# eudald-seeslab/mmsbm

Hardware: NVIDIA B200
Metric: rating-updates/sec (higher is better)
Workload: dtype f64

## Files before the change

mmsbm_b200/csrc/em_step.cu:

```cuda
#include <stdlib.h>

#include "common.cuh"
#include "em_internal.cuh"
#include "segment_pass.cuh"

namespace mmsbm {

constexpr int kPrThreads = 128;
constexpr int kPrBatch = 16;
constexpr int kGemmThreads = 256;
constexpr int kGemmBK = 32;
constexpr int kGemmTR = 4;

__global__ void __launch_bounds__(128) segment_fixup_kernel(const SegArgs A) {
  const int run = blockIdx.y, RNB = A.R * A.NBp;
  const int n_long = __ldg(A.sched + 2);
  const int32_t* long_seg = A.sched + 4 + 3 * A.pmax;
  const int32_t* long_slot0 = long_seg + A.lmax;
  for (int li = blockIdx.x; li < n_long; li += gridDim.x) {
    const int sg = __ldg(long_seg + li), s0 = __ldg(long_slot0 + li), s1 = __ldg(long_slot0 + li + 1);
    MMSBM_DEV_CHECK(sg >= 0 && sg < A.nseg && s0 >= 0 && s0 < s1 && s1 <= A.smax);
    const double* src = A.partial + ((size_t)run * A.smax + s0) * RNB;
    double* dst = A.wg + ((size_t)run * A.nseg + sg) * RNB;
    for (int o = threadIdx.x; o < RNB; o += blockDim.x) {
      double acc = 0.0;
      for (int k = 0; k < s1 - s0; ++k) acc += src[(size_t)k * RNB + o];
      dst[o] = acc;
    }
  }
}

__global__ void interleave_runs_kernel(const double* __restrict__ src, double* __restrict__ dst, int n_src,
                                       int n_dst, int row0, int ld, int group0, int groups, int gs) {
  const int c4 = ld >> 2;
  const size_t total = (size_t)groups * n_src * gs * c4;
  const size_t t = (size_t)blockIdx.x * blockDim.x + threadIdx.x;
  if (t >= total) return;
  const int c = (int)(t % c4);
  const int j = (int)((t / c4) % gs);
  const size_t rest = t / c4 / gs;
  const int id = (int)(rest % n_src);
  const size_t p = group0 + rest / n_src;
  const double4_t v = ldg256(src + (((size_t)(gs * p + j) * n_src + id) * ld + 4 * c));
  stg256(dst + (((p * n_dst + row0 + id) * gs + j) * ld + 4 * c), v);
}

__global__ void prep_p_kernel(const double* pr, int K, int L, int R, int ldk, int ldl, double* pw_u,
                              double* pn_u, double* pw_i, double* pn_i) {
  const int run = blockIdx.y;
  const int total = ldk * ldl * R;
  const int t = blockIdx.x * blockDim.x + threadIdx.x;
  if (t >= total) return;
  const int r = t % R, kl = t / R, lp = kl % ldl, kp = kl / ldl;
  double v = 0.0;
  if (kp < K && lp < L) v = __ldg(pr + (((size_t)run * K + kp) * L + lp) * R + r);
  const size_t base = (size_t)run * total;
  const int rnb_u = R * ldl, rnb_i = R * ldk;
  pw_u[base + (size_t)kp * rnb_u + r * ldl + lp] = v;
  pn_u[base + (size_t)(r * ldl + lp) * ldk + kp] = v;
  pw_i[base + (size_t)lp * rnb_i + r * ldk + kp] = v;
  pn_i[base + (size_t)(r * ldk + kp) * ldl + lp] = v;
}

struct GemmArgs {
  const double* A;
  const double* B;
  double* C;
  const double* own;
  const int32_t* deg;
  int M, N, Kd, lda, rg, normalize;
  int b_resident;
  int bk;
};

template <bool EPI>
__global__ void __launch_bounds__(kGemmThreads) small_gemm_kernel(const GemmArgs g) {
  constexpr int TR = kGemmTR;
  extern __shared__ __align__(32) unsigned char smem_raw[];
  const int BM = TR * g.rg, AS = g.bk + 2;
  double* Bs = reinterpret_cast<double*>(smem_raw);
  double* As = Bs + (size_t)(g.b_resident ? g.Kd : g.bk) * g.N;
  const int run = blockIdx.y;
  const int ncg = g.N >> 2, half = g.N >> 1;
  const int rgid = threadIdx.x / ncg, cg = threadIdx.x - rgid * ncg;
  const bool active = rgid < g.rg;
  const double* A = g.A + (size_t)run * g.M * g.lda;
  const double2* B2 = reinterpret_cast<const double2*>(g.B + (size_t)run * g.Kd * g.N);
  double2* Bs2 = reinterpret_cast<double2*>(Bs);
  if (g.b_resident)
    for (int t = threadIdx.x; t < (g.Kd * g.N) >> 1; t += kGemmThreads) Bs2[t] = __ldg(B2 + t);
  const int n_tiles = (g.M + BM - 1) / BM;
  for (int tile = blockIdx.x; tile < n_tiles; tile += gridDim.x) {
    const int row0 = tile * BM;
    double acc[TR][4];
#pragma unroll
    for (int i = 0; i < TR; ++i)
#pragma unroll
      for (int j = 0; j < 4; ++j) acc[i][j] = 0.0;

    for (int k0 = 0; k0 < g.Kd; k0 += g.bk) {
      const int bk = min(g.bk, g.Kd - k0);
      const int bk2 = bk >> 1;
      __syncthreads();
      for (int t = threadIdx.x; t < BM * bk2; t += kGemmThreads) {
        const int m = t / bk2, p2 = t - m * bk2;
        double2 v = make_double2(0.0, 0.0);
        if (row0 + m < g.M) v = __ldg(reinterpret_cast<const double2*>(A + (size_t)(row0 + m) * g.lda + k0) + p2);
        *reinterpret_cast<double2*>(As + m * AS + 2 * p2) = v;
      }
      if (!g.b_resident)
        for (int t = threadIdx.x; t < (bk * g.N) >> 1; t += kGemmThreads)
          Bs2[t] = __ldg(B2 + (((size_t)k0 * g.N) >> 1) + t);
      __syncthreads();
      if (active) {
        const double* ap = As + (size_t)(TR * rgid) * AS;
        const double* bp = Bs + (size_t)(g.b_resident ? k0 : 0) * g.N + 2 * cg;
        for (int kk = 0; kk < bk; kk += 2) {
          const double2 b00 = *reinterpret_cast<const double2*>(bp + (size_t)kk * g.N);
          const double2 b01 = *reinterpret_cast<const double2*>(bp + (size_t)kk * g.N + half);
          const double2 b10 = *reinterpret_cast<const double2*>(bp + (size_t)(kk + 1) * g.N);
          const double2 b11 = *reinterpret_cast<const double2*>(bp + (size_t)(kk + 1) * g.N + half);
#pragma unroll
          for (int i = 0; i < TR; ++i) {
            const double2 a = *reinterpret_cast<const double2*>(ap + i * AS + kk);
            acc[i][0] = fma(a.x, b00.x, acc[i][0]); acc[i][1] = fma(a.x, b00.y, acc[i][1]);
            acc[i][2] = fma(a.x, b01.x, acc[i][2]); acc[i][3] = fma(a.x, b01.y, acc[i][3]);
            acc[i][0] = fma(a.y, b10.x, acc[i][0]); acc[i][1] = fma(a.y, b10.y, acc[i][1]);
            acc[i][2] = fma(a.y, b11.x, acc[i][2]); acc[i][3] = fma(a.y, b11.y, acc[i][3]);
          }
        }
      }
    }
    if (active) {
#pragma unroll
      for (int i = 0; i < TR; ++i) {
        const int m = row0 + TR * rgid + i;
        if (m >= g.M) continue;
        const size_t off = ((size_t)run * g.M + m) * g.N + 2 * cg;
        double2 v0 = make_double2(acc[i][0], acc[i][1]), v1 = make_double2(acc[i][2], acc[i][3]);
        if (EPI) {
          const double2 o0 = __ldg(reinterpret_cast<const double2*>(g.own + off));
          const double2 o1 = __ldg(reinterpret_cast<const double2*>(g.own + off + half));
          v0.x *= o0.x; v0.y *= o0.y; v1.x *= o1.x; v1.y *= o1.y;
          if (g.normalize) {
            const double d = (double)max(__ldg(g.deg + m), 1);
            v0.x = v0.x / d; v0.y = v0.y / d; v1.x = v1.x / d; v1.y = v1.y / d;
          }
        }
        *reinterpret_cast<double2*>(g.C + off) = v0;
        *reinterpret_cast<double2*>(g.C + off + half) = v1;
      }
    }
  }
}

constexpr int kRowThreads = 256;

template <int LD, int ROWS>
__global__ void __launch_bounds__(kRowThreads) row_w_kernel(const double* __restrict__ own,
                                                            const double* __restrict__ pw,
                                                            double* __restrict__ W, int M, int RNB) {
  extern __shared__ __align__(32) unsigned char smem_raw[];
  double* Ps = reinterpret_cast<double*>(smem_raw);
  const int run = blockIdx.y;
  {
    const double2* src = reinterpret_cast<const double2*>(pw + (size_t)run * LD * RNB);
    double2* dst = reinterpret_cast<double2*>(Ps);
    for (int t = threadIdx.x; t < (LD * RNB) >> 1; t += kRowThreads) dst[t] = __ldg(src + t);
  }
  __syncthreads();
  const double* own_run = own + (size_t)run * M * LD;
  double* w_run = W + (size_t)run * M * RNB;
  for (int m0 = blockIdx.x * (kRowThreads * ROWS) + threadIdx.x; m0 < M; m0 += gridDim.x * (kRowThreads * ROWS)) {
    double o[ROWS][LD];
    int mr[ROWS];
#pragma unroll
    for (int j = 0; j < ROWS; ++j) {
      mr[j] = m0 + j * kRowThreads;
      const int mc = mr[j] < M ? mr[j] : m0;
#pragma unroll
      for (int c = 0; c < LD / 4; ++c) {
        const double4_t v = ldg256(own_run + (size_t)mc * LD + 4 * c);
        o[j][4 * c] = v.x; o[j][4 * c + 1] = v.y; o[j][4 * c + 2] = v.z; o[j][4 * c + 3] = v.w;
      }
    }
    for (int ob = 0; ob < RNB; ob += 4) {
      double4_t acc[ROWS];
#pragma unroll
      for (int j = 0; j < ROWS; ++j) acc[j] = double4_t{0.0, 0.0, 0.0, 0.0};
#pragma unroll
      for (int a = 0; a < LD; ++a) {
        const double4_t p = lds32(Ps + a * RNB + ob);
#pragma unroll
        for (int j = 0; j < ROWS; ++j) {
          acc[j].x = fma(o[j][a], p.x, acc[j].x); acc[j].y = fma(o[j][a], p.y, acc[j].y);
          acc[j].z = fma(o[j][a], p.z, acc[j].z); acc[j].w = fma(o[j][a], p.w, acc[j].w);
        }
      }
#pragma unroll
      for (int j = 0; j < ROWS; ++j)
        if (mr[j] < M) stg256(w_run + (size_t)mr[j] * RNB + ob, acc[j]);
    }
  }
}

template <int LD, int ROWS, int PF>
__global__ void __launch_bounds__(kRowThreads) row_n_kernel(const double* __restrict__ G,
                                                            const double* __restrict__ pn,
                                                            const double* __restrict__ own,
                                                            const int32_t* __restrict__ deg,
                                                            double* __restrict__ out, int M, int RNB,
                                                            int normalize, const RowPublish pub) {
  extern __shared__ __align__(32) unsigned char smem_raw[];
  double* Ps = reinterpret_cast<double*>(smem_raw);
  const int run = blockIdx.y;
  double* pdst = nullptr;
  int pgs = 1, pj = 0;
  size_t pgrp = 0;
#pragma unroll
  for (int t = 0; t < 3; ++t) {
    if (pub.dst[t] != nullptr && run >= pub.gs[t] * pub.group0[t] && run < pub.gs[t] * (pub.group0[t] + pub.groups[t])) {
      pdst = pub.dst[t]; pgs = pub.gs[t]; pgrp = (size_t)(run / pub.gs[t]); pj = run % pub.gs[t];
    }
  }
  {
    const double2* src = reinterpret_cast<const double2*>(pn + (size_t)run * LD * RNB);
    double2* dst = reinterpret_cast<double2*>(Ps);
    for (int t = threadIdx.x; t < (LD * RNB) >> 1; t += kRowThreads) dst[t] = __ldg(src + t);
  }
  __syncthreads();
  const double* g_run = G + (size_t)run * M * RNB;
  const double* own_run = own + (size_t)run * M * LD;
  double* out_run = out + (size_t)run * M * LD;
  for (int m0 = blockIdx.x * (kRowThreads * ROWS) + threadIdx.x; m0 < M; m0 += gridDim.x * (kRowThreads * ROWS)) {
    double acc[ROWS][LD];
    int mr[ROWS];
    const double* grow[ROWS];
#pragma unroll
    for (int j = 0; j < ROWS; ++j) {
      mr[j] = m0 + j * kRowThreads;
      grow[j] = g_run + (size_t)(mr[j] < M ? mr[j] : m0) * RNB;
#pragma unroll
      for (int a = 0; a < LD; ++a) acc[j][a] = 0.0;
    }
    for (int ob0 = 0; ob0 < RNB; ob0 += 4 * PF) {
      double4_t gq[ROWS][PF];
#pragma unroll
      for (int j = 0; j < ROWS; ++j)
#pragma unroll
        for (int p = 0; p < PF; ++p) gq[j][p] = ldg256(grow[j] + ob0 + 4 * p);
#pragma unroll
      for (int p = 0; p < PF; ++p) {
        const int ob = ob0 + 4 * p;
        double gv[ROWS][4];
#pragma unroll
        for (int j = 0; j < ROWS; ++j) {
          gv[j][0] = gq[j][p].x; gv[j][1] = gq[j][p].y; gv[j][2] = gq[j][p].z; gv[j][3] = gq[j][p].w;
        }
#pragma unroll
        for (int i = 0; i < 4; ++i) {
#pragma unroll
          for (int c = 0; c < LD / 4; ++c) {
            const double4_t pv = lds32(Ps + (ob + i) * LD + 4 * c);
#pragma unroll
            for (int j = 0; j < ROWS; ++j) {
              acc[j][4 * c] = fma(gv[j][i], pv.x, acc[j][4 * c]);         acc[j][4 * c + 1] = fma(gv[j][i], pv.y, acc[j][4 * c + 1]);
              acc[j][4 * c + 2] = fma(gv[j][i], pv.z, acc[j][4 * c + 2]); acc[j][4 * c + 3] = fma(gv[j][i], pv.w, acc[j][4 * c + 3]);
            }
          }
        }
      }
    }
#pragma unroll
    for (int j = 0; j < ROWS; ++j) {
      if (mr[j] >= M) continue;
      double d = 1.0;
      if (normalize) d = (double)max(__ldg(deg + mr[j]), 1);
#pragma unroll
      for (int c = 0; c < LD / 4; ++c) {
        const double4_t ov = ldg256(own_run + (size_t)mr[j] * LD + 4 * c);
        double4_t v{acc[j][4 * c] * ov.x, acc[j][4 * c + 1] * ov.y, acc[j][4 * c + 2] * ov.z, acc[j][4 * c + 3] * ov.w};
        if (normalize) { v.x = v.x / d; v.y = v.y / d; v.z = v.z / d; v.w = v.w / d; }
        stg256(out_run + (size_t)mr[j] * LD + 4 * c, v);
        if (pdst) stg256(pdst + (((pgrp * pub.n_all + pub.row0 + mr[j]) * pgs + pj) * LD + 4 * c), v);
      }
    }
  }
}

struct PrArgs {
  const double* own;
  const double* g;
  double* partial;
  int nseg, NA, lda, RNB;
};

__global__ void __launch_bounds__(kPrThreads) pr_accumulate_kernel(const PrArgs A) {
  extern __shared__ __align__(32) unsigned char smem_raw[];
  double* own_s = reinterpret_cast<double*>(smem_raw);
  double* g_s = own_s + kPrBatch * A.lda;
  const int run = blockIdx.y, slab = blockIdx.x;
  const int per = (A.nseg + kPrSlabs - 1) / kPrSlabs;
  const int s0 = slab * per, s1 = min(s0 + per, A.nseg);
  const int nout = A.NA * A.RNB;
  const int ta = A.lda >> 2, tb = A.RNB >> 2, n_tiles = ta * tb;
  const double* own_run = A.own + (size_t)run * A.nseg * A.lda;
  const double* g_run = A.g + (size_t)run * A.nseg * A.RNB;
  double* dst = A.partial + ((size_t)run * kPrSlabs + slab) * nout;

  for (int tile0 = 0; tile0 < n_tiles; tile0 += kPrThreads) {
    const int tile = tile0 + threadIdx.x;
    const bool on = tile < n_tiles;
    const int a0 = on ? 4 * (tile / tb) : 0, b0 = on ? 4 * (tile % tb) : 0;
    double acc[4][4];
#pragma unroll
    for (int i = 0; i < 4; ++i)
#pragma unroll
      for (int k = 0; k < 4; ++k) acc[i][k] = 0.0;
    for (int c0 = s0; c0 < s1; c0 += kPrBatch) {
      const int nb = min(kPrBatch, s1 - c0);
      __syncthreads();
      {
        const double2* src = reinterpret_cast<const double2*>(own_run + (size_t)c0 * A.lda);
        double2* d2 = reinterpret_cast<double2*>(own_s);
        for (int t = threadIdx.x; t < (nb * A.lda) >> 1; t += kPrThreads) d2[t] = __ldg(src + t);
        src = reinterpret_cast<const double2*>(g_run + (size_t)c0 * A.RNB);
        d2 = reinterpret_cast<double2*>(g_s);
        for (int t = threadIdx.x; t < (nb * A.RNB) >> 1; t += kPrThreads) d2[t] = __ldg(src + t);
      }
      __syncthreads();
      if (on) {
        for (int sg = 0; sg < nb; ++sg) {
          const double4_t o = lds32(own_s + sg * A.lda + a0);
          const double4_t g = lds32(g_s + sg * A.RNB + b0);
          const double ov[4] = {o.x, o.y, o.z, o.w};
#pragma unroll
          for (int i = 0; i < 4; ++i) {
            acc[i][0] = fma(ov[i], g.x, acc[i][0]); acc[i][1] = fma(ov[i], g.y, acc[i][1]);
            acc[i][2] = fma(ov[i], g.z, acc[i][2]); acc[i][3] = fma(ov[i], g.w, acc[i][3]);
          }
        }
      }
    }
    if (on) {
#pragma unroll
      for (int i = 0; i < 4; ++i)
        if (a0 + i < A.NA)
          stg256(dst + (size_t)(a0 + i) * A.RNB + b0, double4_t{acc[i][0], acc[i][1], acc[i][2], acc[i][3]});
    }
  }
}

struct PrFinArgs {
  const double* partial;
  const double* pr;
  double* pr_out;
  int K, L, R, NA, NBp, transposed, normalize;
};

constexpr int kFinWarps = 8;
__global__ void __launch_bounds__(kFinWarps * 32) pr_finalize_kernel(const PrFinArgs A) {
  extern __shared__ __align__(16) unsigned char smem_raw[];
  const int run = blockIdx.y, a = blockIdx.x;
  const int RNB = A.R * A.NBp, nout = A.NA * RNB;
  double* part_s = reinterpret_cast<double*>(smem_raw);
  double* tot_s = part_s + kFinWarps * RNB;
  const int lane = threadIdx.x & 31, warp = threadIdx.x >> 5;
  const double* part = A.partial + (size_t)run * kPrSlabs * nout + (size_t)a * RNB;
  constexpr int per = kPrSlabs / kFinWarps;
  for (int o = lane; o < RNB; o += 32) {
    double acc = 0.0;
#pragma unroll 4
    for (int s = warp * per; s < (warp + 1) * per; ++s) acc += part[(size_t)s * nout + o];
    part_s[warp * RNB + o] = acc;
  }
  __syncthreads();
  for (int o = threadIdx.x; o < RNB; o += blockDim.x) {
    double acc = 0.0;
    for (int w = 0; w < kFinWarps; ++w) acc += part_s[w * RNB + o];
    tot_s[o] = acc;
  }
  __syncthreads();
  const int NB = A.transposed ? A.K : A.L;
  for (int b = threadIdx.x; b < NB; b += blockDim.x) {
    const int k = A.transposed ? b : a, l = A.transposed ? a : b;
    const size_t kl = (size_t)k * A.L + l;
    const double* prs = A.pr + ((size_t)run * A.K * A.L + kl) * A.R;
    double* dst = A.pr_out + ((size_t)run * A.K * A.L + kl) * A.R;
    double tot = 0.0;
    for (int r = 0; r < A.R; ++r) {
      const double v = tot_s[r * A.NBp + b] * prs[r];
      dst[r] = v;
      tot += v;
    }
    if (A.normalize) {
      const double d = (tot == 0.0) ? 1.0 : tot;
      for (int r = 0; r < A.R; ++r) dst[r] = dst[r] / d;
    }
  }
}

__global__ void finalize_eta_kernel(double* eta, const int32_t* deg, int n_items, int ldl, int L,
                                    size_t total) {
  size_t t = (size_t)blockIdx.x * blockDim.x + threadIdx.x;
  if (t >= total) return;
  int col = (int)(t % ldl);
  size_t row = t / ldl;
  int item = (int)(row % n_items);
  if (col < L) eta[t] = eta[t] / (double)max(__ldg(deg + item), 1);
}

__global__ void finalize_pr_kernel(double* pr, int KL_total, int R) {
  int t = blockIdx.x * blockDim.x + threadIdx.x;
  if (t >= KL_total) return;
  double* row = pr + (size_t)t * R;
  double tot = 0.0;
  for (int r = 0; r < R; ++r) tot += row[r];
  const double d = (tot == 0.0) ? 1.0 : tot;
  for (int r = 0; r < R; ++r) row[r] = row[r] / d;
}

struct PassShape { int G, CH, UN, MINB; };

int env_int(const char* name, int dflt) {
  const char* v = getenv(name);
  return (v && *v) ? atoi(v) : dflt;
}

int sm_count() {
  static int cached[64] = {0};
  int dev = 0;
  if (cudaGetDevice(&dev) != cudaSuccess || dev < 0 || dev >= 64) return 148;
  if (cached[dev] == 0) {
    int n = 0;
    if (cudaDeviceGetAttribute(&n, cudaDevAttrMultiProcessorCount, dev) != cudaSuccess || n <= 0) n = 148;
    cached[dev] = n;
  }
// ... 29 lines not shown
static bool pairs_enabled(int NBp, int R, int n_runs) {
  return n_runs >= 2 && NBp <= 32 && seg_smem_bytes(R, NBp, 2) <= kMaxSmemBytes && env_int("MMSBM_PAIR", 1) != 0;
}

static int g_reserved_ctas = 0;
void set_reserved_ctas(int n) { g_reserved_ctas = n > 0 ? n : 0; }

static unsigned grid_x_for(const SegArgs& a, int ctas_per_sm) {
  if (!a.counters) return (unsigned)((a.pmax + a.segs_per_cta - 1) / a.segs_per_cta);
  int64_t resident = (int64_t)sm_count() * ctas_per_sm - g_reserved_ctas;
  if (resident < 1) resident = 1;
  const int64_t want = (a.pmax + kWarps - 1) / kWarps;
  return (unsigned)(want < resident ? want : resident);
}

static bool hexa_enabled(int NBp, int R, int n_runs) {
  return n_runs >= 6 && NBp == 20 && seg_smem_bytes(R, NBp, 6) <= kMaxSmemBytes && env_int("MMSBM_HEXA", 1) != 0;
}

RunPlan plan_runs(int NBp, int R, int n_runs, bool hexa_table) {
  RunPlan p{0, 0, 0, 0};
  if (hexa_table && hexa_enabled(NBp, R, n_runs)) p.hexas = n_runs / 6;
  p.single_from = 6 * p.hexas;
  if (pairs_enabled(NBp, R, n_runs - p.single_from)) {
    p.pairs = (n_runs - p.single_from) / 2;
    p.pair_group0 = p.single_from / 2;
    p.single_from += 2 * p.pairs;
  }
  return p;
}

static int launch_segment_pass_impl(SegArgs a, const double* nbr_pairs, const double* nbr_hexa,
                                    int64_t n_ratings, int n_runs, cudaStream_t st) {
  const double avg_degree = (double)n_ratings / (double)a.nseg;
  PassShape sh = choose_shape(a.NBp, avg_degree);
  const int un_e = env_int("MMSBM_UN", 0), occ_e = env_int("MMSBM_OCC", 0);
  const RunPlan plan = plan_runs(a.NBp, a.R, n_runs, nbr_hexa != nullptr);
  const int single_from = plan.single_from;
  if (plan.hexas > 0) {
    const int hexas = plan.hexas;
    SegArgs p = a;
    p.nbr = nbr_hexa;
    p.run_base = 0;
    p.grp_base = 0;
    p.segs_per_cta = segs_per_cta_for(a.pmax, n_ratings, hexas);
    const unsigned gx = grid_x_for(p, occ_e > 0 ? occ_e : 3);
    if (p.counters) a.counters += hexas;
    const size_t smem = seg_smem_bytes(a.R, a.NBp, 6);
    int rc = MMSBM_ERANGE;
    if (un_e > 0 || occ_e > 0)
      rc = launch_segment_pass_hexa(p, sh.G, un_e > 0 ? un_e : 3, occ_e > 0 ? occ_e : 3, dim3(gx, hexas), smem, st);
    if (rc == MMSBM_ERANGE) rc = launch_segment_pass_hexa(p, sh.G, 3, 3, dim3(gx, hexas), smem, st);
    if (rc) {
      if (rc == MMSBM_ERANGE) set_error("no six-run segment-pass variant for G=%d", sh.G);
      return rc;
    }
    if (single_from == n_runs && plan.pairs == 0) return 0;
  }
  if (plan.pairs > 0) {
    MMSBM_REQUIRE(nbr_pairs, MMSBM_EINVAL, "segment pass: the table of run pairs is missing");
    const int pairs = plan.pairs;
    SegArgs p = a;
    p.nbr = nbr_pairs;
    p.run_base = 6 * plan.hexas;
    p.grp_base = plan.pair_group0;
    p.counters = a.counters;
    p.segs_per_cta = segs_per_cta_for(a.pmax, n_ratings, pairs);
    const unsigned gx = grid_x_for(p, occ_e > 0 ? occ_e : 3);
    if (p.counters) a.counters += pairs;
    const size_t smem = seg_smem_bytes(a.R, a.NBp, 2);
    int UN = (sh.G == 1) ? 2 : 3, MINB = 3;
    int rc = MMSBM_ERANGE;
    if (un_e > 0 || occ_e > 0)
      rc = launch_segment_pass_pair(p, sh.G, un_e > 0 ? un_e : UN, occ_e > 0 ? occ_e : MINB, dim3(gx, pairs), smem, st);
    if (rc == MMSBM_ERANGE) rc = launch_segment_pass_pair(p, sh.G, UN, MINB, dim3(gx, pairs), smem, st);
    if (rc == MMSBM_ERANGE && sh.G == 1) rc = launch_segment_pass_pair(p, sh.G, 2, 3, dim3(gx, pairs), smem, st);
    if (rc) {
      if (rc == MMSBM_ERANGE) set_error("no paired segment-pass variant for G=%d", sh.G);
      return rc;
    }
  }
  if (single_from == n_runs) return 0;
  a.run_base = single_from;
  a.segs_per_cta = segs_per_cta_for(a.pmax, n_ratings, n_runs - single_from);
  const unsigned gx = grid_x_for(a, occ_e > 0 ? occ_e : sh.MINB);
  const dim3 grid(gx, n_runs - single_from);
  const size_t smem = seg_smem_bytes(a.R, a.NBp, 1);
  MMSBM_REQUIRE(smem <= kMaxSmemBytes, MMSBM_ERANGE,
                "segment pass needs %zu bytes of shared memory (R=%d, row stride %d)", smem, a.R, a.NBp);
  auto go = [&](const PassShape& p) {
    switch (p.CH) {
      case 1: return launch_segment_pass_ch1(a, p.G, p.UN, p.MINB, grid, smem, st);
      case 2: return launch_segment_pass_ch2(a, p.G, p.UN, p.MINB, grid, smem, st);
      case 4: return launch_segment_pass_ch4(a, p.G, p.UN, p.MINB, grid, smem, st);
      default: return launch_segment_pass_ch8(a, p.G, p.UN, p.MINB, grid, smem, st);
    }
  };
  if (un_e > 0 || occ_e > 0) {
    PassShape alt = sh;
    if (un_e > 0) alt.UN = un_e;
    if (occ_e > 0) alt.MINB = occ_e;
    const int rc = go(alt);
    if (rc != MMSBM_ERANGE) return rc;
  }
  const int rc = go(sh);
  if (rc == MMSBM_ERANGE) set_error("no segment-pass variant for G=%d CH=%d UN=%d", sh.G, sh.CH, sh.UN);
  return rc;
}

int launch_segment_pass_and_fixup(SegArgs a, const double* nbr_pairs, const double* nbr_hexa,
                                  int64_t n_ratings, int n_runs, cudaStream_t st, bool no_long_segments) {
  int rc = launch_segment_pass_impl(a, nbr_pairs, nbr_hexa, n_ratings, n_runs, st);
  if (rc) return rc;
  if (no_long_segments) return 0;
  const int64_t fix_ctas = 4 * sm_count();
  const unsigned gx = (unsigned)(a.lmax < fix_ctas ? a.lmax : fix_ctas);
  segment_fixup_kernel<<<dim3(gx, n_runs), 128, 0, st>>>(a);
  MMSBM_LAUNCH_CHECK("segment_fixup_kernel");
  return 0;
}

template <bool EPI>
static int launch_gemm(GemmArgs g, int n_runs, cudaStream_t st) {
  const int ncg = g.N / 4;
  MMSBM_REQUIRE(g.N % 4 == 0 && g.Kd % 4 == 0 && ncg >= 1 && ncg <= kGemmThreads, MMSBM_ERANGE,
                "small gemm: N=%d Kd=%d not supported (N <= 1024, multiples of 4)", g.N, g.Kd);
  int rg = kGemmThreads / ncg;
  if (rg > 32) rg = 32;
  g.rg = rg;
  const int BM = kGemmTR * rg;
  g.bk = kGemmBK;
  size_t smem = ((size_t)g.Kd * g.N + (size_t)BM * (g.bk + 2)) * 8;
  g.b_resident = smem <= 200 * 1024;
  if (!g.b_resident) {
    auto slab_bytes = [&](int bk) { return ((size_t)bk * g.N + (size_t)BM * (bk + 2)) * 8; };
    while (g.bk > 4 && slab_bytes(g.bk) > kMaxSmemBytes) g.bk -= 4;
    smem = slab_bytes(g.bk);
  }
  MMSBM_REQUIRE(smem <= kMaxSmemBytes, MMSBM_ERANGE,
                "small gemm needs %zu bytes of shared memory (K*L*R too large)", smem);
  auto kern = small_gemm_kernel<EPI>;
  MMSBM_CUDA(cudaFuncSetAttribute(kern, cudaFuncAttributeMaxDynamicSharedMemorySize, (int)smem));
  const int n_tiles = (g.M + BM - 1) / BM;
  int per_run = (sm_count() * 3 + n_runs - 1) / n_runs;
  if (per_run > n_tiles) per_run = n_tiles;
  if (per_run < 1) per_run = 1;
  kern<<<dim3(per_run, n_runs), kGemmThreads, smem, st>>>(g);
  MMSBM_LAUNCH_CHECK("small_gemm_kernel");
  return 0;
}

int launch_w(const double* own, const double* pw, double* W, int M, int LD, int RNB, int n_runs,
             cudaStream_t st) {
  const size_t smem = (size_t)LD * RNB * 8;
  const int rows_env = env_int("MMSBM_ROWS", 2);
#define MMSBM_ROW_W(LDv)                                                                        \
  if (LD == LDv && smem <= 200 * 1024) {                                                        \
    constexpr int kRows = (LDv <= 24) ? 2 : 1;             \
    const bool two = kRows == 2 && rows_env == 2;                                               \
    auto kern = two ? row_w_kernel<LDv, kRows> : row_w_kernel<LDv, 1>;                          \
    const int per = kRowThreads * (two ? 2 : 1);                                                \
    const int gx = min((M + per - 1) / per, sm_count() * 2);                                           \
    MMSBM_CUDA(cudaFuncSetAttribute(kern, cudaFuncAttributeMaxDynamicSharedMemorySize, (int)smem)); \
    kern<<<dim3(gx, n_runs), kRowThreads, smem, st>>>(own, pw, W, M, RNB);                      \
    MMSBM_LAUNCH_CHECK("row_w_kernel");                                                         \
    return 0;                                                                                   \
  }
  MMSBM_ROW_W(4) MMSBM_ROW_W(8) MMSBM_ROW_W(12) MMSBM_ROW_W(16) MMSBM_ROW_W(20) MMSBM_ROW_W(24)
  MMSBM_ROW_W(28) MMSBM_ROW_W(32)
#undef MMSBM_ROW_W
  GemmArgs g{own, pw, W, nullptr, nullptr, M, RNB, LD, LD, 0, 0, 0, kGemmBK};
  return launch_gemm<false>(g, n_runs, st);
}

int launch_n(const double* G, const double* pn, const double* own, const int32_t* deg, double* out,
             int M, int LD, int RNB, int normalize, int n_runs, cudaStream_t st, const RowPublish* publish) {
  const size_t smem = (size_t)LD * RNB * 8;
  RowPublish pub{};
  if (publish) pub = *publish;
  const int rows_env = env_int("MMSBM_ROWS_N", 1);
  int pf = env_int("MMSBM_ROWN_PF", 5);
  if (pf != 1 && pf != 2 && pf != 5) pf = 1;
  if ((RNB / 4) % pf != 0) pf = ((RNB / 4) % 2 == 0 && pf != 1) ? 2 : 1;
#define MMSBM_ROW_N_GO(kern, two)                                                               \
  {                                                                                             \
    const int per = kRowThreads * ((two) ? 2 : 1);                                              \
    const int gx = min((M + per - 1) / per, sm_count() * 2);                                    \
    MMSBM_CUDA(cudaFuncSetAttribute(kern, cudaFuncAttributeMaxDynamicSharedMemorySize, (int)smem)); \
    kern<<<dim3(gx, n_runs), kRowThreads, smem, st>>>(G, pn, own, deg, out, M, RNB, normalize, pub); \
    MMSBM_LAUNCH_CHECK("row_n_kernel");                                                         \
    return 0;                                                                                   \
  }
#define MMSBM_ROW_N(LDv)                                                                        \
  if (LD == LDv && smem <= 200 * 1024) {                                                        \
    constexpr int kRows = (LDv <= 24) ? 2 : 1;         \
    const bool two = kRows == 2 && rows_env == 2;                                               \
    if (two) MMSBM_ROW_N_GO((row_n_kernel<LDv, kRows, 1>), true)                                \
    if (pf == 5) MMSBM_ROW_N_GO((row_n_kernel<LDv, 1, 5>), false)                               \
    if (pf == 2) MMSBM_ROW_N_GO((row_n_kernel<LDv, 1, 2>), false)                               \
    MMSBM_ROW_N_GO((row_n_kernel<LDv, 1, 1>), false)                                            \
  }
  MMSBM_ROW_N(4) MMSBM_ROW_N(8) MMSBM_ROW_N(12) MMSBM_ROW_N(16) MMSBM_ROW_N(20) MMSBM_ROW_N(24)
  MMSBM_ROW_N(28) MMSBM_ROW_N(32)
#undef MMSBM_ROW_N_GO
#undef MMSBM_ROW_N
  GemmArgs g{G, pn, out, own, deg, M, LD, RNB, RNB, 0, normalize, 0, kGemmBK};
  int rc = launch_gemm<true>(g, n_runs, st);
  if (rc || !publish) return rc;
  for (int t = 0; t < 3; ++t)
    if (pub.dst[t] && (rc = launch_interleave(out, pub.dst[t], M, pub.n_all, pub.row0, LD, pub.group0[t],
                                              pub.groups[t], pub.gs[t], st)))
      return rc;
  return 0;
}

int launch_prep_p(const double* pr, int K, int L, int R, int ldk, int ldl, int n_runs, double* pw_u,
                  double* pn_u, double* pw_i, double* pn_i, cudaStream_t st) {
  const int total = ldk * ldl * R;
  prep_p_kernel<<<dim3((total + 255) / 256, n_runs), 256, 0, st>>>(pr, K, L, R, ldk, ldl, pw_u, pn_u, pw_i, pn_i);
  MMSBM_LAUNCH_CHECK("prep_p_kernel");
  return 0;
}

int launch_interleave(const double* src, double* dst, int n_src, int n_dst, int row0, int ld, int group0,
                      int groups, int gs, cudaStream_t st) {
  const size_t tot = (size_t)groups * n_src * gs * (ld / 4);
  if (tot == 0) return 0;
  interleave_runs_kernel<<<(unsigned)((tot + 255) / 256), 256, 0, st>>>(src, dst, n_src, n_dst, row0, ld,
                                                                        group0, groups, gs);
  MMSBM_LAUNCH_CHECK("interleave_runs_kernel");
  return 0;
}

int launch_pr(const double* own, const double* g, double* partial, const double* pr, double* pr_out,
              int nseg, int NA, int lda, int NBp, int K, int L, int R, int n_runs, bool transposed,
              bool normalize, cudaStream_t st) {
  PrArgs pa{};
  pa.own = own; pa.g = g; pa.partial = partial;
  pa.nseg = nseg; pa.NA = NA; pa.lda = lda; pa.RNB = R * NBp;
  const size_t smem = (size_t)kPrBatch * (pa.lda + pa.RNB) * 8;
  MMSBM_CUDA(cudaFuncSetAttribute(pr_accumulate_kernel, cudaFuncAttributeMaxDynamicSharedMemorySize,
                                  (int)smem));
  pr_accumulate_kernel<<<dim3(kPrSlabs, n_runs), kPrThreads, smem, st>>>(pa);
  MMSBM_LAUNCH_CHECK("pr_accumulate_kernel");
  PrFinArgs fa{};
  fa.partial = partial; fa.pr = pr; fa.pr_out = pr_out;
  fa.K = K; fa.L = L; fa.R = R; fa.NA = NA; fa.NBp = NBp;
  fa.transposed = transposed ? 1 : 0;
  fa.normalize = normalize ? 1 : 0;
  const size_t fin_smem = (size_t)(kFinWarps + 1) * R * NBp * 8;
  MMSBM_CUDA(cudaFuncSetAttribute(pr_finalize_kernel, cudaFuncAttributeMaxDynamicSharedMemorySize, (int)fin_smem));
  pr_finalize_kernel<<<dim3(NA, n_runs), kFinWarps * 32, fin_smem, st>>>(fa);
  MMSBM_LAUNCH_CHECK("pr_finalize_kernel");
  return 0;
}

int launch_finalize_pr(double* pr, int kl_total, int R, cudaStream_t st) {
  finalize_pr_kernel<<<(kl_total + 127) / 128, 128, 0, st>>>(pr, kl_total, R);
  MMSBM_LAUNCH_CHECK("finalize_pr_kernel");
  return 0;
}

struct EmDims {
  int U, I, R, K, L, S, ldk, ldl, rnb_u, rnb_i;
  bool emit_items;
  int nseg_e, NA_e, NBp_e;
  size_t p_elems, wg_u_elems, wg_i_elems, partial_elems, slots_u_elems, slots_i_elems;
  size_t th2_elems, et2_elems;
  size_t et6_elems;
  size_t ctr_elems;
  int64_t lmax, smax, pmax_u, pmax_i;
};

static EmDims em_dims(int64_t N, int U, int I, int R, int K, int L, int S) {
  EmDims d;
  d.U = U; d.I = I; d.R = R; d.K = K; d.L = L; d.S = S;
  d.ldk = row_stride(K); d.ldl = row_stride(L);
  d.rnb_u = R * d.ldl; d.rnb_i = R * d.ldk;
  d.emit_items = (I <= U);
  d.nseg_e = d.emit_items ? I : U;
  d.NA_e = d.emit_items ? L : K;
  d.NBp_e = d.emit_items ? d.ldk : d.ldl;
  d.p_elems = (size_t)S * d.ldk * d.ldl * R;
  d.wg_u_elems = (size_t)S * U * d.rnb_u;
  d.wg_i_elems = (size_t)S * I * d.rnb_i;
  d.partial_elems = (size_t)S * kPrSlabs * d.NA_e * R * d.NBp_e;
  d.lmax = N / MMSBM_PIECE_LEN + 1;
  d.smax = 2 * (N / MMSBM_PIECE_LEN) + 1;
  d.pmax_u = (int64_t)U + N / MMSBM_PIECE_LEN + 1;
  d.pmax_i = (int64_t)I + N / MMSBM_PIECE_LEN + 1;
  d.slots_u_elems = (size_t)S * d.smax * d.rnb_u;
  d.slots_i_elems = (size_t)S * d.smax * d.rnb_i;
  d.th2_elems = (size_t)(S / 2) * 2 * U * d.ldk;
  d.et2_elems = (size_t)(S / 2) * 2 * I * d.ldl;
  d.et6_elems = (size_t)(S / 6) * 6 * I * d.ldl;
  d.ctr_elems = 2 * ((size_t)S + 8);
  return d;
}

static size_t em_main_bytes(const EmDims& d) {
  return 4 * align_up(d.p_elems * 8) + align_up(d.wg_u_elems * 8) + align_up(d.wg_i_elems * 8) +
         align_up(d.partial_elems * 8) + align_up(d.slots_u_elems * 8) + align_up(d.slots_i_elems * 8) +
         align_up(d.th2_elems * 8) + align_up(d.et2_elems * 8) + align_up(d.et6_elems * 8) + align_up(d.ctr_elems * 4) + 256;
}

}

using namespace mmsbm;

extern "C" int mmsbm_em_workspace_bytes(int64_t N, int32_t U, int32_t I, int32_t R, int32_t K,
                                        int32_t L, int32_t S, size_t* bytes) {
  MMSBM_REQUIRE(bytes && N >= 0 && U > 0 && I > 0 && R > 0 && K > 0 && L > 0 && S > 0, MMSBM_EINVAL,
                "mmsbm_em_workspace_bytes: bad argument");
  EmDims d = em_dims(N, U, I, R, K, L, S);
  *bytes = em_main_bytes(d);
  if (em_small_applicable(N, R, K, L, S)) *bytes += align_up(em_small_partial_elems(R, K) * 8);
  return 0;
}

struct Overlap {
  bool no_long_u = false, no_long_i = false;
  cudaStream_t side = nullptr;
  cudaEvent_t e[6] = {nullptr, nullptr, nullptr, nullptr, nullptr, nullptr};
  bool two_branch = false;
};

static int em_step_impl(const int32_t* useg, const int32_t* uadj, const int32_t* udeg,
                        const int32_t* iseg, const int32_t* iadj, const int32_t* ideg,
                        const int32_t* usched, const int32_t* isched, int64_t N, int32_t U, int32_t I, int32_t R, int32_t K, int32_t L,
                        int32_t S, const double* theta, const double* eta, const double* pr,
                        double* theta_out, double* eta_out, double* pr_out, int32_t flags,
                        void* ws, size_t ws_bytes, void* stream, cudaEvent_t* ev,
                        const Overlap* ov = nullptr) {
  MMSBM_REQUIRE(useg && uadj && udeg && iseg && iadj && ideg && usched && isched && theta && eta && pr &&
                    theta_out && eta_out && pr_out && ws, MMSBM_EINVAL, "mmsbm_em_step: null pointer");
  MMSBM_REQUIRE(N >= 0 && U > 0 && I > 0 && R > 0 && K > 0 && L > 0 && S > 0, MMSBM_EINVAL,
                "mmsbm_em_step: bad size");
  MMSBM_REQUIRE(K <= 256 && L <= 256 && R <= 31, MMSBM_ERANGE,
                "mmsbm_em_step: K, L <= 256 and R <= 31 supported (K=%d L=%d R=%d)", K, L, R);
  cudaStream_t st = static_cast<cudaStream_t>(stream);
  EmDims d = em_dims(N, U, I, R, K, L, S);
  const RunPlan plan_u = plan_runs(d.ldl, R, S, true), plan_i = plan_runs(d.ldk, R, S, false);
  Arena arena(ws, ws_bytes);
  double* pw_u = arena.take<double>(d.p_elems);
  double* pn_u = arena.take<double>(d.p_elems);
  double* pw_i = arena.take<double>(d.p_elems);
  double* pn_i = arena.take<double>(d.p_elems);
  double* wg_u = arena.take<double>(d.wg_u_elems);
  double* wg_i = arena.take<double>(d.wg_i_elems);
  double* partial = arena.take<double>(d.partial_elems);
  double* slots_u = arena.take<double>(d.slots_u_elems);
  double* slots_i = arena.take<double>(d.slots_i_elems);
  double* th2 = arena.take<double>(d.th2_elems);
  double* et2 = arena.take<double>(d.et2_elems);
  double* et6 = arena.take<double>(d.et6_elems);
  int32_t* counters = arena.take<int32_t>(d.ctr_elems);
  MMSBM_REQUIRE(pw_u && pn_u && pw_i && pn_i && wg_u && wg_i && partial && slots_u && slots_i && th2 && et2 && et6 && counters,
// ... 231 lines not shown
```

Before: 26.45 billion.

## Use FP64 DMMA tensor cores in row_w and row_n kernels

Rewrites the per-row small-GEMM kernels (own×Pw and G×Pn) to issue m8n8k4 FP64 mma.sync instead of scalar DFMA loops. The P matrices are restaged in shared memory in fragment order, and each warp processes 8-row tiles. row_n also software-prefetches the next 16-wide K chunk of G. It adds a DMMA vs DFMA microbenchmark and drops the env-selected ROWS/prefetch variants. In exchange the global accesses become narrower and strided per lane, and the shared-memory footprint grows with padding.

Measured after the change: 27.08 billion, median of 6. 2.4% higher.

```diff
diff --git a/mmsbm_b200/csrc/em_step.cu b/mmsbm_b200/csrc/em_step.cu
--- a/mmsbm_b200/csrc/em_step.cu
+++ b/mmsbm_b200/csrc/em_step.cu
@@ -154,66 +154,80 @@
   }
 }
 
+__device__ __forceinline__ void dmma(double2& d, double a, double b) {
+  asm("mma.sync.aligned.m8n8k4.row.col.f64.f64.f64.f64 {%0,%1}, {%2}, {%3}, {%0,%1};"
+      : "+d"(d.x), "+d"(d.y) : "d"(a), "d"(b));
+}
+
 constexpr int kRowThreads = 256;
-
-template <int LD, int ROWS>
+constexpr int kRowWarps = kRowThreads / 32;
+constexpr int kRowTilesW = 4;
+constexpr int kRowTilesN = 2;
+
+static size_t row_w_smem(int LD, int RNB) { return (size_t)LD * ((RNB + 7) & ~7) * 8; }
+static size_t row_n_smem(int LD, int RNB) { return (size_t)((RNB + 15) & ~15) * ((LD + 7) & ~7) * 8; }
+
+template <int LD, int TW>
 __global__ void __launch_bounds__(kRowThreads) row_w_kernel(const double* __restrict__ own,
                                                             const double* __restrict__ pw,
                                                             double* __restrict__ W, int M, int RNB) {
+  constexpr int KS = LD / 4;
   extern __shared__ __align__(32) unsigned char smem_raw[];
-  double* Ps = reinterpret_cast<double*>(smem_raw);
-  const int run = blockIdx.y;
+  double* Bs = reinterpret_cast<double*>(smem_raw);
+  const int run = blockIdx.y, lane = threadIdx.x & 31, warp = threadIdx.x >> 5;
+  const int qr = lane >> 2, qc = lane & 3;
+  const int NT = (RNB + 7) >> 3;
   {
-    const double2* src = reinterpret_cast<const double2*>(pw + (size_t)run * LD * RNB);
-    double2* dst = reinterpret_cast<double2*>(Ps);
-    for (int t = threadIdx.x; t < (LD * RNB) >> 1; t += kRowThreads) dst[t] = __ldg(src + t);
+    const double* src = pw + (size_t)run * LD * RNB;
+    for (int t = threadIdx.x; t < KS * NT * 32; t += kRowThreads) {
+      const int l = t & 31, f = t >> 5, nt = f % NT, s = f / NT, o = 8 * nt + (l >> 2);
+      Bs[t] = o < RNB ? __ldg(src + (size_t)(4 * s + (l & 3)) * RNB + o) : 0.0;
+    }
   }
   __syncthreads();
   const double* own_run = own + (size_t)run * M * LD;
   double* w_run = W + (size_t)run * M * RNB;
-  for (int m0 = blockIdx.x * (kRowThreads * ROWS) + threadIdx.x; m0 < M; m0 += gridDim.x * (kRowThreads * ROWS)) {
-    double o[ROWS][LD];
-    int mr[ROWS];
-#pragma unroll
-    for (int j = 0; j < ROWS; ++j) {
-      mr[j] = m0 + j * kRowThreads;
-      const int mc = mr[j] < M ? mr[j] : m0;
-#pragma unroll
-      for (int c = 0; c < LD / 4; ++c) {
-        const double4_t v = ldg256(own_run + (size_t)mc * LD + 4 * c);
-        o[j][4 * c] = v.x; o[j][4 * c + 1] = v.y; o[j][4 * c + 2] = v.z; o[j][4 * c + 3] = v.w;
+  for (int m0 = (blockIdx.x * kRowWarps + warp) * 8 * TW; m0 < M; m0 += gridDim.x * kRowWarps * 8 * TW) {
+    double a[TW][KS];
+#pragma unroll
+    for (int t = 0; t < TW; ++t) {
+      const int m = m0 + 8 * t + qr;
+#pragma unroll
+      for (int s = 0; s < KS; ++s) a[t][s] = m < M ? __ldg(own_run + (size_t)m * LD + 4 * s + qc) : 0.0;
+    }
+    for (int nt = 0; nt < NT; ++nt) {
+      double2 acc[TW];
+#pragma unroll
+      for (int t = 0; t < TW; ++t) acc[t] = make_double2(0.0, 0.0);
+#pragma unroll
+      for (int s = 0; s < KS; ++s) {
+        const double b = Bs[(s * NT + nt) * 32 + lane];
+#pragma unroll
+        for (int t = 0; t < TW; ++t) dmma(acc[t], a[t][s], b);
       }
-    }
-    for (int ob = 0; ob < RNB; ob += 4) {
-      double4_t acc[ROWS];
-#pragma unroll
-      for (int j = 0; j < ROWS; ++j) acc[j] = double4_t{0.0, 0.0, 0.0, 0.0};
-#pragma unroll
-      for (int a = 0; a < LD; ++a) {
-        const double4_t p = lds32(Ps + a * RNB + ob);
-#pragma unroll
-        for (int j = 0; j < ROWS; ++j) {
-          acc[j].x = fma(o[j][a], p.x, acc[j].x); acc[j].y = fma(o[j][a], p.y, acc[j].y);
-          acc[j].z = fma(o[j][a], p.z, acc[j].z); acc[j].w = fma(o[j][a], p.w, acc[j].w);
-        }
+      const int o = 8 * nt + 2 * qc;
+#pragma unroll
+      for (int t = 0; t < TW; ++t) {
+        const int m = m0 + 8 * t + qr;
+        if (m < M && o < RNB) *reinterpret_cast<double2*>(w_run + (size_t)m * RNB + o) = acc[t];
       }
-#pragma unroll
-      for (int j = 0; j < ROWS; ++j)
-        if (mr[j] < M) stg256(w_run + (size_t)mr[j] * RNB + ob, acc[j]);
-    }
-  }
-}
-
-template <int LD, int ROWS, int PF>
+    }
+  }
+}
+
+template <int LD, int TN>
 __global__ void __launch_bounds__(kRowThreads) row_n_kernel(const double* __restrict__ G,
                                                             const double* __restrict__ pn,
                                                             const double* __restrict__ own,
                                                             const int32_t* __restrict__ deg,
                                                             double* __restrict__ out, int M, int RNB,
                                                             int normalize, const RowPublish pub) {
+  constexpr int NT = (LD + 7) / 8;
   extern __shared__ __align__(32) unsigned char smem_raw[];
-  double* Ps = reinterpret_cast<double*>(smem_raw);
-  const int run = blockIdx.y;
+  double* Bs = reinterpret_cast<double*>(smem_raw);
+  const int run = blockIdx.y, lane = threadIdx.x & 31, warp = threadIdx.x >> 5;
+  const int qr = lane >> 2, qc = lane & 3;
+  const int KC = (RNB + 15) >> 4;
   double* pdst = nullptr;
   int pgs = 1, pj = 0;
   size_t pgrp = 0;
@@ -224,65 +238,73 @@
     }
   }
   {
-    const double2* src = reinterpret_cast<const double2*>(pn + (size_t)run * LD * RNB);
-    double2* dst = reinterpret_cast<double2*>(Ps);
-    for (int t = threadIdx.x; t < (LD * RNB) >> 1; t += kRowThreads) dst[t] = __ldg(src + t);
+    const double* src = pn + (size_t)run * LD * RNB;
+    for (int t = threadIdx.x; t < KC * 4 * NT * 32; t += kRowThreads) {
+      const int l = t & 31, f = t >> 5, nt = f % NT, cj = f / NT;
+      const int k = 16 * (cj >> 2) + 4 * (l & 3) + (cj & 3), n = 8 * nt + (l >> 2);
+      Bs[t] = (k < RNB && n < LD) ? __ldg(src + (size_t)k * LD + n) : 0.0;
+    }
   }
   __syncthreads();
   const double* g_run = G + (size_t)run * M * RNB;
   const double* own_run = own + (size_t)run * M * LD;
   double* out_run = out + (size_t)run * M * LD;
-  for (int m0 = blockIdx.x * (kRowThreads * ROWS) + threadIdx.x; m0 < M; m0 += gridDim.x * (kRowThreads * ROWS)) {
-    double acc[ROWS][LD];
-    int mr[ROWS];
-    const double* grow[ROWS];
-#pragma unroll
-    for (int j = 0; j < ROWS; ++j) {
-      mr[j] = m0 + j * kRowThreads;
-      grow[j] = g_run + (size_t)(mr[j] < M ? mr[j] : m0) * RNB;
-#pragma unroll
-      for (int a = 0; a < LD; ++a) acc[j][a] = 0.0;
-    }
-    for (int ob0 = 0; ob0 < RNB; ob0 += 4 * PF) {
-      double4_t gq[ROWS][PF];
-#pragma unroll
-      for (int j = 0; j < ROWS; ++j)
-#pragma unroll
-        for (int p = 0; p < PF; ++p) gq[j][p] = ldg256(grow[j] + ob0 + 4 * p);
-#pragma unroll
-      for (int p = 0; p < PF; ++p) {
-        const int ob = ob0 + 4 * p;
-        double gv[ROWS][4];
-#pragma unroll
-        for (int j = 0; j < ROWS; ++j) {
-          gv[j][0] = gq[j][p].x; gv[j][1] = gq[j][p].y; gv[j][2] = gq[j][p].z; gv[j][3] = gq[j][p].w;
-        }
-#pragma unroll
-        for (int i = 0; i < 4; ++i) {
-#pragma unroll
-          for (int c = 0; c < LD / 4; ++c) {
-            const double4_t pv = lds32(Ps + (ob + i) * LD + 4 * c);
-#pragma unroll
-            for (int j = 0; j < ROWS; ++j) {
-              acc[j][4 * c] = fma(gv[j][i], pv.x, acc[j][4 * c]);         acc[j][4 * c + 1] = fma(gv[j][i], pv.y, acc[j][4 * c + 1]);
-              acc[j][4 * c + 2] = fma(gv[j][i], pv.z, acc[j][4 * c + 2]); acc[j][4 * c + 3] = fma(gv[j][i], pv.w, acc[j][4 * c + 3]);
-            }
+  const double4_t zero{0.0, 0.0, 0.0, 0.0};
+  for (int m0 = (blockIdx.x * kRowWarps + warp) * 8 * TN; m0 < M; m0 += gridDim.x * kRowWarps * 8 * TN) {
+    const double* grow[TN];
+    bool live[TN];
+    double2 acc[TN][NT];
+#pragma unroll
+    for (int t = 0; t < TN; ++t) {
+      const int m = m0 + 8 * t + qr;
+      live[t] = m < M;
+      grow[t] = g_run + (size_t)(live[t] ? m : 0) * RNB + 4 * qc;
+#pragma unroll
+      for (int nt = 0; nt < NT; ++nt) acc[t][nt] = make_double2(0.0, 0.0);
+    }
+    double4_t x[TN], y[TN];
+#pragma unroll
+    for (int t = 0; t < TN; ++t) {
+      x[t] = (live[t] && 4 * qc < RNB) ? ldg256(grow[t]) : zero;
+      y[t] = zero;
+    }
+    for (int c = 0; c < KC; ++c) {
+      if (c + 1 < KC) {
+        const bool in = 16 * (c + 1) + 4 * qc < RNB;
+#pragma unroll
+        for (int t = 0; t < TN; ++t) y[t] = (live[t] && in) ? ldg256(grow[t] + 16 * (c + 1)) : zero;
+      }
+      const double* bc = Bs + (size_t)c * 4 * NT * 32 + lane;
+#pragma unroll
+      for (int j = 0; j < 4; ++j) {
+#pragma unroll
+        for (int nt = 0; nt < NT; ++nt) {
+          const double b = bc[(j * NT + nt) * 32];
+#pragma unroll
+          for (int t = 0; t < TN; ++t) {
+            const double a = j == 0 ? x[t].x : j == 1 ? x[t].y : j == 2 ? x[t].z : x[t].w;
+            dmma(acc[t][nt], a, b);
           }
         }
       }
-    }
-#pragma unroll
-    for (int j = 0; j < ROWS; ++j) {
-      if (mr[j] >= M) continue;
+#pragma unroll
+      for (int t = 0; t < TN; ++t) x[t] = y[t];
+    }
+#pragma unroll
+    for (int t = 0; t < TN; ++t) {
+      const int m = m0 + 8 * t + qr;
+      if (m >= M) continue;
       double d = 1.0;
-      if (normalize) d = (double)max(__ldg(deg + mr[j]), 1);
-#pragma unroll
-      for (int c = 0; c < LD / 4; ++c) {
-        const double4_t ov = ldg256(own_run + (size_t)mr[j] * LD + 4 * c);
-        double4_t v{acc[j][4 * c] * ov.x, acc[j][4 * c + 1] * ov.y, acc[j][4 * c + 2] * ov.z, acc[j][4 * c + 3] * ov.w};
-        if (normalize) { v.x = v.x / d; v.y = v.y / d; v.z = v.z / d; v.w = v.w / d; }
-        stg256(out_run + (size_t)mr[j] * LD + 4 * c, v);
-        if (pdst) stg256(pdst + (((pgrp * pub.n_all + pub.row0 + mr[j]) * pgs + pj) * LD + 4 * c), v);
+      if (normalize) d = (double)max(__ldg(deg + m), 1);
+#pragma unroll
+      for (int nt = 0; nt < NT; ++nt) {
+        const int col = 8 * nt + 2 * qc;
+        if (col >= LD) continue;
+        const double2 ov = __ldg(reinterpret_cast<const double2*>(own_run + (size_t)m * LD + col));
+        double2 v = make_double2(acc[t][nt].x * ov.x, acc[t][nt].y * ov.y);
+        if (normalize) { v.x = v.x / d; v.y = v.y / d; }
+        *reinterpret_cast<double2*>(out_run + (size_t)m * LD + col) = v;
+        if (pdst) *reinterpret_cast<double2*>(pdst + ((pgrp * pub.n_all + pub.row0 + m) * pgs + pj) * LD + col) = v;
       }
     }
   }
@@ -618,15 +640,12 @@
 
 int launch_w(const double* own, const double* pw, double* W, int M, int LD, int RNB, int n_runs,
              cudaStream_t st) {
-  const size_t smem = (size_t)LD * RNB * 8;
-  const int rows_env = env_int("MMSBM_ROWS", 2);
+  const size_t smem = row_w_smem(LD, RNB);
 #define MMSBM_ROW_W(LDv)                                                                        \
-  if (LD == LDv && smem <= 200 * 1024) {                                                        \
-    constexpr int kRows = (LDv <= 24) ? 2 : 1;             \
-    const bool two = kRows == 2 && rows_env == 2;                                               \
-    auto kern = two ? row_w_kernel<LDv, kRows> : row_w_kernel<LDv, 1>;                          \
-    const int per = kRowThreads * (two ? 2 : 1);                                                \
-    const int gx = min((M + per - 1) / per, sm_count() * 2);                                           \
+  if (LD == LDv && smem <= kMaxSmemBytes) {                                                     \
+    auto kern = row_w_kernel<LDv, kRowTilesW>;                                                  \
+    const int per = kRowWarps * 8 * kRowTilesW;                                                 \
+    const int gx = min((M + per - 1) / per, sm_count() * 2);                                    \
     MMSBM_CUDA(cudaFuncSetAttribute(kern, cudaFuncAttributeMaxDynamicSharedMemorySize, (int)smem)); \
     kern<<<dim3(gx, n_runs), kRowThreads, smem, st>>>(own, pw, W, M, RNB);                      \
     MMSBM_LAUNCH_CHECK("row_w_kernel");                                                         \
@@ -641,34 +660,21 @@
 
 int launch_n(const double* G, const double* pn, const double* own, const int32_t* deg, double* out,
              int M, int LD, int RNB, int normalize, int n_runs, cudaStream_t st, const RowPublish* publish) {
-  const size_t smem = (size_t)LD * RNB * 8;
+  const size_t smem = row_n_smem(LD, RNB);
   RowPublish pub{};
   if (publish) pub = *publish;
-  const int rows_env = env_int("MMSBM_ROWS_N", 1);
-  int pf = env_int("MMSBM_ROWN_PF", 5);
-  if (pf != 1 && pf != 2 && pf != 5) pf = 1;
-  if ((RNB / 4) % pf != 0) pf = ((RNB / 4) % 2 == 0 && pf != 1) ? 2 : 1;
-#define MMSBM_ROW_N_GO(kern, two)                                                               \
-  {                                                                                             \
-    const int per = kRowThreads * ((two) ? 2 : 1);                                              \
+#define MMSBM_ROW_N(LDv)                                                                        \
+  if (LD == LDv && smem <= kMaxSmemBytes) {                                                     \
+    auto kern = row_n_kernel<LDv, kRowTilesN>;                                                  \
+    const int per = kRowWarps * 8 * kRowTilesN;                                                 \
     const int gx = min((M + per - 1) / per, sm_count() * 2);                                    \
     MMSBM_CUDA(cudaFuncSetAttribute(kern, cudaFuncAttributeMaxDynamicSharedMemorySize, (int)smem)); \
     kern<<<dim3(gx, n_runs), kRowThreads, smem, st>>>(G, pn, own, deg, out, M, RNB, normalize, pub); \
     MMSBM_LAUNCH_CHECK("row_n_kernel");                                                         \
     return 0;                                                                                   \
   }
-#define MMSBM_ROW_N(LDv)                                                                        \
-  if (LD == LDv && smem <= 200 * 1024) {                                                        \
-    constexpr int kRows = (LDv <= 24) ? 2 : 1;         \
-    const bool two = kRows == 2 && rows_env == 2;                                               \
-    if (two) MMSBM_ROW_N_GO((row_n_kernel<LDv, kRows, 1>), true)                                \
-    if (pf == 5) MMSBM_ROW_N_GO((row_n_kernel<LDv, 1, 5>), false)                               \
-    if (pf == 2) MMSBM_ROW_N_GO((row_n_kernel<LDv, 1, 2>), false)                               \
-    MMSBM_ROW_N_GO((row_n_kernel<LDv, 1, 1>), false)                                            \
-  }
   MMSBM_ROW_N(4) MMSBM_ROW_N(8) MMSBM_ROW_N(12) MMSBM_ROW_N(16) MMSBM_ROW_N(20) MMSBM_ROW_N(24)
   MMSBM_ROW_N(28) MMSBM_ROW_N(32)
-#undef MMSBM_ROW_N_GO
 #undef MMSBM_ROW_N
   GemmArgs g{G, pn, out, own, deg, M, LD, RNB, RNB, 0, normalize, 0, kGemmBK};
   int rc = launch_gemm<true>(g, n_runs, st);
diff --git a/profiles/microbench/dmma_bench.cu b/profiles/microbench/dmma_bench.cu
--- /dev/null
+++ b/profiles/microbench/dmma_bench.cu
@@ -0,0 +1,100 @@
+#include <cuda_runtime.h>
+#include <stdio.h>
+
+constexpr int ITERS = 4096;
+
+__device__ __forceinline__ void dmma(double& d0, double& d1, double a, double b) {
+  asm volatile("mma.sync.aligned.m8n8k4.row.col.f64.f64.f64.f64 {%0,%1}, {%2}, {%3}, {%0,%1};"
+               : "+d"(d0), "+d"(d1) : "d"(a), "d"(b));
+}
+
+template <int CH>
+__global__ void dmma_kernel(double* out, long long* cycles, double a, double b) {
+  double c0[CH], c1[CH];
+#pragma unroll
+  for (int i = 0; i < CH; ++i) { c0[i] = threadIdx.x * 1e-9 + i; c1[i] = 0.5 * i; }
+  const long long t0 = clock64();
+  for (int it = 0; it < ITERS; ++it) {
+#pragma unroll
+    for (int i = 0; i < CH; ++i) dmma(c0[i], c1[i], a, b);
+  }
+  const long long t1 = clock64();
+  double s = 0.0;
+#pragma unroll
+  for (int i = 0; i < CH; ++i) s += c0[i] + c1[i];
+  out[blockIdx.x * blockDim.x + threadIdx.x] = s;
+  if (threadIdx.x == 0) cycles[blockIdx.x] = t1 - t0;
+}
+
+template <int CH>
+__global__ void dfma_kernel(double* out, long long* cycles, double a, double b) {
+  double c[CH];
+#pragma unroll
+  for (int i = 0; i < CH; ++i) c[i] = threadIdx.x * 1e-9 + i;
+  const long long t0 = clock64();
+  for (int it = 0; it < ITERS; ++it) {
+#pragma unroll
+    for (int i = 0; i < CH; ++i) asm volatile("fma.rn.f64 %0, %1, %2, %0;" : "+d"(c[i]) : "d"(a), "d"(b));
+  }
+  const long long t1 = clock64();
+  double s = 0.0;
+#pragma unroll
+  for (int i = 0; i < CH; ++i) s += c[i];
+  out[blockIdx.x * blockDim.x + threadIdx.x] = s;
+  if (threadIdx.x == 0) cycles[blockIdx.x] = t1 - t0;
+}
+
+template <typename K>
+static void run(const char* name, K kern, int ch, int fma_per_warp_op, int warps_per_sm, int sms, double* out,
+                long long* cyc) {
+  const int threads = 32 * (warps_per_sm < 32 ? warps_per_sm : 32);
+  const int blocks_per_sm = warps_per_sm * 32 / threads;
+  const int blocks = sms * blocks_per_sm;
+  cudaEvent_t e0, e1;
+  cudaEventCreate(&e0);
+  cudaEventCreate(&e1);
+  kern<<<blocks, threads>>>(out, cyc, 1.0000001, 1e-7);
+  cudaEventRecord(e0);
+  kern<<<blocks, threads>>>(out, cyc, 1.0000001, 1e-7);
+  cudaEventRecord(e1);
+  cudaEventSynchronize(e1);
+  float ms = 0.f;
+  cudaEventElapsedTime(&ms, e0, e1);
+  long long h[4096];
+  cudaMemcpy(h, cyc, sizeof(long long) * blocks, cudaMemcpyDeviceToHost);
+  long long mx = 0;
+  for (int i = 0; i < blocks; ++i) mx = h[i] > mx ? h[i] : mx;
+  const double fma_per_sm = (double)warps_per_sm * ITERS * ch * fma_per_warp_op;
+  const double total_fma = fma_per_sm * sms;
+  printf("%-5s chains/warp=%d warps/SM=%2d  %7.1f FMA/clk/SM  %6.3f ms  %6.2f TFLOP/s  (%.0f MHz effective)\n", name,
+         ch, warps_per_sm, fma_per_sm / (double)mx, ms, 2.0 * total_fma / (ms * 1e-3) / 1e12,
+         (double)mx / (ms * 1e-3) / 1e6);
+  cudaEventDestroy(e0);
+  cudaEventDestroy(e1);
+}
+
+int main() {
+  cudaDeviceProp p;
+  cudaGetDeviceProperties(&p, 0);
+  const int sms = p.multiProcessorCount;
+  printf("%s, %d SMs\n", p.name, sms);
+  double* out;
+  long long* cyc;
+  cudaMalloc(&out, sizeof(double) * sms * 1024 * 2);
+  cudaMalloc(&cyc, sizeof(long long) * 4096);
+  for (int w : {1, 4, 8, 16, 32}) {
+    run("DMMA", dmma_kernel<1>, 1, 256, w, sms, out, cyc);
+    run("DMMA", dmma_kernel<2>, 2, 256, w, sms, out, cyc);
+    run("DMMA", dmma_kernel<4>, 4, 256, w, sms, out, cyc);
+    run("DMMA", dmma_kernel<8>, 8, 256, w, sms, out, cyc);
+    run("DFMA", dfma_kernel<1>, 1, 32, w, sms, out, cyc);
+    run("DFMA", dfma_kernel<4>, 4, 32, w, sms, out, cyc);
+    run("DFMA", dfma_kernel<8>, 8, 32, w, sms, out, cyc);
+  }
+  const cudaError_t e = cudaDeviceSynchronize();
+  if (e != cudaSuccess) {
+    printf("error: %s\n", cudaGetErrorString(e));
+    return 1;
+  }
+  return 0;
+}
```
